# balint256/gr-baz

Measured on AMD Instinct MI355X. Metric: MUSIC-DoA snapshots/s (4 ant, 1024 samp, 3600 bins), higher is better.
Workload: dtype f64; 1 GPU; cfg2 (BASELINE.json configs[1]): m=4 n=2 nsamples=1024 (K=256) resolution=3600, spectrum port wired, 8 streams x 32768 items per GPU per step, device-resident; streams_total=8, items_per_launch_sequence=262144, parallelism=independent streams, s mod 1, no collective, collective_backend_fell_back=False

## Files before the change

### gr_baz_amd/csrc/baz_music_hip.hip

```cpp
#include "../../include/baz_music_hip.h"
#include "music_kernels.hip.h"
#include "music_wide_kernels.hip.h"
#include "scan_coarse_kernels.hip.h"
#include "scan_i8_kernels.hip.h"
#ifdef BAZ_MUSIC_LAB
#include "scan_i8p_kernels.hip.h"
#include "sort_kernels.hip.h"
#endif
#include "table_kernels.hip.h"
#include "smoothing_kernels.hip.h"
#include "refine_kernels.hip.h"
#include "average_kernels.hip.h"

#include <algorithm>
#include <chrono>
#include <cmath>
#include <cstdio>
#include <cstdlib>
#include <cstring>
#include <unistd.h>
#include <mutex>
#include <thread>
#include <new>
#include <string>
// ... 174 lines not shown
    uint32_t wide_cap = 0;
    double* dSs = nullptr;
    int sig_scan = 1;
    uint8_t* dRedo = nullptr;
    int sub_evd = 1;
    int fused_covevd = 0;
    uint32_t covevd_blocks = 512u;
    int covevd_task_items = 0;
    uint32_t cov4_resident_blocks = 256u;
    uint32_t cs_tiles = 0;
    int coarse = 1;
    int coarse_rg = 4;
    int coarse_lab = 0;
    int coarse_stats = 0;
    unsigned long long* dMargin = nullptr;
#ifdef BAZ_MUSIC_LAB
    uint16_t* dKeys = nullptr;
    uint32_t* dHist = nullptr;
    uint32_t* dCursor = nullptr;
    uint32_t* dPerm = nullptr;
    uint32_t sort_cap = 0;
    unsigned long long* dFire = nullptr;
    unsigned long long* hFire = nullptr;
    unsigned long long* hFireDev = nullptr;
    unsigned long long fire_calls = 0, fire_seen = 0;
    int sort_mode = 0;
    bool sort_on = false;
    uint32_t sort_streak = 0;
    uint64_t sort_clock = 0, sort_retry_at = 0;
    double rate_unsorted = 0.0;
    uint64_t sorted_calls = 0, unsorted_calls = 0;
#endif
    uint32_t scan_lds_pad = 0;
    int seq_walk = 0;
#ifdef BAZ_MUSIC_LAB
    int i8p_on = 0;
#endif
    int i8_on = 1;
    int i8_abl = 0;
    int refine_nocount = 0;
    uint32_t num_cus = 256;
    int i8_wgs_per_cu[2][2][2] = {{{0, 0}, {0, 0}}, {{0, 0}, {0, 0}}};
    unsigned long long* dI8Stat = nullptr;
    int peak_mode = 0;
    float* dPeakSpec = nullptr;
    size_t peak_spec_cap = 0;
    int order_mode = 0;
    uint32_t order_nsnap = 0;
    uint8_t* dOrd = nullptr;
    size_t ord_cap = 0;
    uint32_t ord_count = 0;
    uint32_t ord_items = 0;
    bool ord_on = false;
    bool ord_driven = false;
    uint8_t* ord_cur = nullptr;
    uint8_t* dOrdTap = nullptr;
    size_t ord_tap_cap = 0;
    int refine_mode = 0;
    float* dRefAl = nullptr;
    size_t ref_al_cap = 0;
    double* dRefOff = nullptr;
    size_t ref_off_cap = 0;
    uint32_t ref_count = 0;
    bool ref_on = false;
    uint32_t avg_window = 1;
    double avg_beta = 1.0;
    double avg_neff = 1.0;
    bazavg::AvgTable avg_tab = {};
    uint32_t avg_hist = 0;
    int avg_parity = 0;
    double2* dAvgHist[2] = {nullptr, nullptr};
    size_t avg_hist_cap[2] = {0, 0};
    double2* dRavg = nullptr;
    size_t ravg_cap = 0;
    size_t chunk_bytes = 0;
    struct HostPin { uintptr_t lo, hi; uint32_t asked; };
    std::vector<HostPin> pins;
    std::vector<HostPin> refused;
    uint64_t pinned_bytes = 0;
    uint64_t pin_limit = 4096ull << 20;
    int auto_pin = 0;
    int zero_copy = 1;
    int single_limit_mib = 64;
    StageProf prof[BAZ_MUSIC_NUM_STAGES];
    std::string stage_name[BAZ_MUSIC_NUM_STAGES];
    char scan_names[4][64] = {{0}, {0}, {0}, {0}};
    int scan_kind = -1;
    char hip_err[256] = {0};
    struct Smoothing {
        baz_music_ctx* inner = nullptr;
        uint32_t ms = 0, L = 1, Kp = 0;
        int fb = 0;
        bazsmooth::Perm perm = {};
        float2* dY = nullptr;
        size_t y_cap = 0;
        float* dX = nullptr;
        float* dAl = nullptr;
        float* dSpec = nullptr;
        size_t x_cap = 0, al_cap = 0, spec_cap = 0;
    } sm;
};

namespace {

int hip_fail(baz_music_ctx* c, hipError_t e, const char* what)
{
    if (c) snprintf(c->hip_err, sizeof(c->hip_err), "%s: %s", what, hipGetErrorString(e));
    (void)hipGetLastError();
    return BAZ_MUSIC_E_HIP;
}

#define HIP_TRY(ctx, call)                                         \
    do {                                                           \
        hipError_t e__ = (call);                                   \
        if (e__ != hipSuccess) return hip_fail((ctx), e__, #call); \
    } while (0)

struct DeviceGuard {
    int prev = -1;
// ... 526 lines not shown

int launch_frontend(baz_music_ctx* c, const void* d_in, uint32_t batch, double* dQ, uint32_t qstride)
{
    const float* in = static_cast<const float*>(d_in);
    if (c->avg_window > 1) {
        int ra = launch_cov(c, in, batch, c->dR);
        if (ra == BAZ_MUSIC_OK) ra = launch_average(c, c->dR, batch, c->dRavg);
        return ra ? ra : launch_evd(c, c->dRavg, batch, dQ, qstride, c->dG);
    }
    if (c->fused_covevd) return launch_covevd(c, in, batch, dQ, qstride, c->dG);
    const int r = launch_cov(c, in, batch, c->dR);
    return r ? r : launch_evd(c, c->dR, batch, dQ, qstride, c->dG);
}

uint32_t topn_list_len(uint32_t n) { return n <= 2 ? 2u : (n <= 4 ? 4u : (n <= 8 ? 8u : 16u)); }
uint32_t forced_nsplit(int force_nsplit, uint32_t most) { return std::max<uint32_t>(1u, std::min<uint32_t>((uint32_t)force_nsplit, most)); }

struct ScanGeom { uint32_t groups, nsplit, blocks, rows_per_class; };
constexpr uint32_t SCAN_WANT_TASKS = 256u * 4u * 4u * 2u;
constexpr uint32_t SCAN_MAX_NSPLIT = 64;
ScanGeom scan_geometry(uint32_t batch, uint32_t nsteps, uint32_t nclass, int force_nsplit, uint32_t m)
{
    ScanGeom G;
    G.rows_per_class = round_up((batch + nclass - 1) / nclass, 64);
    G.groups = nclass * (G.rows_per_class / 16);
    const uint32_t live_groups = (batch + 15) / 16;
    const uint32_t want_tasks = (m >= 9) ? SCAN_WANT_TASKS / 4u : SCAN_WANT_TASKS;
    const uint32_t ns = (want_tasks + live_groups - 1) / live_groups;
    G.nsplit = std::max<uint32_t>(1u, std::min<uint32_t>(ns, std::min<uint32_t>(nsteps, SCAN_MAX_NSPLIT)));
    if (force_nsplit > 0) G.nsplit = forced_nsplit(force_nsplit, std::min<uint32_t>(nsteps, SCAN_MAX_NSPLIT));
    G.blocks = (G.groups / 4) * G.nsplit;
    return G;
}
size_t scan_cand_ranges(const baz_music_ctx* c, uint32_t batch)
{
    const size_t cap_split = std::min<size_t>(SCAN_MAX_NSPLIT, std::max<uint32_t>(1u, c->fb_steps));
    const size_t exact = (size_t)batch * scan_geometry(batch, c->fb_steps, c->nclass, c->force_nsplit, c->m).nsplit;
    const size_t worst = std::min<size_t>((size_t)batch * cap_split, (size_t)16u * SCAN_WANT_TASKS + (size_t)batch);
    const size_t forced = c->force_nsplit > 0 ? (size_t)batch * forced_nsplit(c->force_nsplit, (uint32_t)cap_split) : 0;
    return std::max(std::max(exact, worst), std::max(forced, (size_t)batch));
}

constexpr uint32_t I8_MAX_NSPLIT = 16, I8_MAX_ROUNDS = 8;
uint32_t i8_nsplit(uint32_t batch, uint32_t nsteps, uint32_t slots, int force_nsplit)
{
    const uint32_t groups = std::max<uint32_t>(1u, (batch + 63) / 64);
    const uint32_t cap = std::max<uint32_t>(1u, std::min<uint32_t>(I8_MAX_NSPLIT, nsteps / 4));
    if (force_nsplit > 0) return forced_nsplit(force_nsplit, std::min<uint32_t>(nsteps, SCAN_MAX_NSPLIT));
    uint32_t best = 1;
    double best_fill = 0.0;
    for (uint32_t r = 1; r <= I8_MAX_ROUNDS; ++r) {
        const uint32_t ns = std::max<uint32_t>(1u, std::min<uint32_t>(cap, (uint32_t)(((uint64_t)r * slots) / groups)));
        const uint64_t blocks = (uint64_t)groups * ns;
        const uint64_t rounds = (blocks + slots - 1) / slots;
        const double fill = (double)blocks / (double)(rounds * slots);
        if (fill > best_fill * 1.03) { best_fill = fill; best = ns; }
        if (ns == cap) break;
    }
    return best;
}
size_t i8_cand_ranges(const baz_music_ctx* c, uint32_t batch)
{
    if (!c->tab.dIB) return 0;
    const size_t exact = (size_t)batch * (c->force_nsplit > 0 ? forced_nsplit(c->force_nsplit, SCAN_MAX_NSPLIT) : I8_MAX_NSPLIT);
    return std::max(exact, std::min<size_t>((size_t)batch * I8_MAX_NSPLIT, (size_t)64u * I8_MAX_ROUNDS * 4u * c->num_cus + (size_t)batch));
}
// ... 98 lines not shown
}

template <int M>
int launch_sort_t(baz_music_ctx* c, const double* dQ, uint32_t qstride, uint32_t batch)
{
    if constexpr (M <= 8) {
        const uint32_t ns = bazsort::key_samples(c->res);
        const uint32_t padded = round_up(batch, 256);
        hipLaunchKernelGGL((bazsort::coarse_key_kernel<M>), dim3(padded / 256), dim3(256), 0, c->stream, dQ, c->tab.dKT, ns, batch, qstride, c->dKeys);
        HIP_TRY(c, hipGetLastError());
        hipLaunchKernelGGL((bazsort::key_sweep_kernel<false>), dim3(bazsort::KEY_BLOCKS), dim3(256), 0, c->stream, c->dKeys, padded / 8, c->dHist,
                           c->dCursor, c->dPerm);
        HIP_TRY(c, hipGetLastError());
        hipLaunchKernelGGL((bazsort::key_sweep_kernel<true>), dim3(bazsort::KEY_BLOCKS), dim3(256), 0, c->stream, c->dKeys, padded / 8, c->dHist,
                           c->dCursor, c->dPerm);
        HIP_TRY(c, hipGetLastError());
    }
    return BAZ_MUSIC_OK;
}
#endif

ScanRefine scan_refine(const baz_music_ctx* c, bool a2)
{
    ScanRefine rf;
    rf.Gs = c->refine_off ? nullptr : c->dG;
    rf.TB = c->tab.dTB + c->tb_step_elems;
    rf.below = c->tab.refine_below;
    rf.count = c->refine_nocount ? nullptr : c->dRefined + c->stat_parity;
    rf.A2 = (a2 && c->tab.dA2p) ? c->tab.dA2p + 64 : nullptr;
    return rf;
}
ScanRefine scan_refine_validation(const baz_music_ctx* c) { return {nullptr, c->tab.dTB + c->tb_step_elems, 0.0, nullptr, nullptr}; }

enum ScanKind { SCAN_FP64 = 0, SCAN_I8 = 1, SCAN_COARSE = 2, SCAN_I8P = 3 };
struct ScanForm { ScanKind kind; bool short_form; };

ScanForm scan_form(const baz_music_ctx* c, bool spec)
{
    if (!spec && coarse_applies(c) && !c->order_mode) return {SCAN_COARSE, false};
    if (spec && i8p_active(c)) return {SCAN_I8P, false};
    const bool gated_shape = c->m <= 8 && !short_form_applies(c->m, c->n);
    if (i8_active(c) && (spec || !gated_shape)) return {SCAN_I8, false};
    return {SCAN_FP64, short_form_in_use(c)};
}

struct ScanCall { uint32_t batch, qstride; float* spec; bool vec4; };

struct ScanDone {
    int rc;
    ScanKind kind;
    uint32_t nsplit;
#ifdef BAZ_MUSIC_LAB
    bool sorted = false;
#endif
};
ScanDone scan_result(baz_music_ctx* c, ScanDone done, int rc) { done.rc = rc; if (rc == BAZ_MUSIC_OK) c->scan_kind = done.kind; return done; }
int launch_rc(baz_music_ctx* c) { HIP_TRY(c, hipGetLastError()); return BAZ_MUSIC_OK; }
ScanDone scan_no_kernel(ScanKind kind) { return {BAZ_MUSIC_E_UNSUPPORTED, kind, 1}; }
struct CoarseLaunch {
    uint32_t blocks, nphases, nsplit;
    ScanRefine rf;
    unsigned long long* stats;
    float* val_dump = nullptr;
    const uint32_t* perm = nullptr;
    unsigned long long* fstat = nullptr;
};
template <int M, typename Kernel>
void coarse_launch(baz_music_ctx* c, Kernel kernel, const CoarseLaunch& L, uint32_t batch, uint32_t qstride)
{
    hipLaunchKernelGGL(kernel, dim3(L.blocks), dim3(256), 0, c->stream, c->dQ, c->tab.dCS, c->tab.dCS + (size_t)(c->cs_tiles + 1) * cs_c_units(M),
                       c->dCand, batch, c->res, qstride, L.nphases, L.nsplit, c->keep_mask, c->n, L.rf, c->tab.cs, L.stats, L.val_dump, L.perm, L.fstat);
}

struct I8Launch {
    uint32_t blocks, nsplit, n;
    float* spec;
// ... 100 lines not shown
        ScanDone done{BAZ_MUSIC_OK, SCAN_I8P, G.nsplit};
        if ((size_t)s.batch * G.nsplit * NMAX > c->cand_cap) return scan_result(c, done, BAZ_MUSIC_E_INVALID);
        const I8Launch L{G.blocks, G.nsplit, c->n, s.spec, scan_refine(c, false), c->dI8Stat, nullptr};
        auto* kernel = s.vec4 ? &scan_i8p_kernel<M, NMAX, true, true> : &scan_i8p_kernel<M, NMAX, true, false>;
        if constexpr (M == 4 && NMAX == 2) {
            if (s.vec4 && c->i8_abl) {
                switch (c->i8_abl) {
                    case 1: kernel = &scan_i8p_kernel<M, NMAX, true, true, false, 1>; break;
                    case 2: kernel = &scan_i8p_kernel<M, NMAX, true, true, false, 2>; break;
                    case 4: kernel = &scan_i8p_kernel<M, NMAX, true, true, false, 4>; break;
                    case 5: kernel = &scan_i8p_kernel<M, NMAX, true, true, false, 5>; break;
                    default: kernel = &scan_i8p_kernel<M, NMAX, true, true, false, 3>; break;
                }
            }
        }
        i8p_launch(c, kernel, L, G.rows_per_class, s.batch, s.qstride);
        return scan_result(c, done, launch_rc(c));
    }
    return scan_no_kernel(SCAN_I8P);
}
#else
template <int M, int NMAX>
ScanDone launch_scan_i8p(baz_music_ctx*, const ScanCall&) { return scan_no_kernel(SCAN_I8P); }
#endif

template <int M, int NMAX, int SIG>
auto* scan_fp64_kernel(const ScanCall& s)
{
    if (s.vec4) return &scan_mfma_kernel<M, NMAX, true, true, 0, (1 | 2 | 16), SIG>;
    if (s.spec) return &scan_mfma_kernel<M, NMAX, true, false, 0, (1 | 2 | 16), SIG>;
    return &scan_mfma_kernel<M, NMAX, false, false, 0, (1 | 2 | 16), SIG>;
}

template <int M, int NMAX>
ScanDone launch_scan_fp64(baz_music_ctx* c, const ScanCall& s, bool short_form)
{
    const ScanGeom G = scan_geometry(s.batch, c->fb_steps, c->nclass, c->force_nsplit, c->m);
    ScanDone done{BAZ_MUSIC_OK, SCAN_FP64, G.nsplit};
    if ((size_t)s.batch * G.nsplit * NMAX > c->cand_cap) return scan_result(c, done, BAZ_MUSIC_E_INVALID);
    auto* kernel = scan_fp64_kernel<M, NMAX, 0>(s);
    if constexpr (M >= 6 && NMAX == 2) {
        if (short_form && c->n == 1) kernel = scan_fp64_kernel<M, NMAX, 1>(s);
        if constexpr (M >= 9) if (short_form && c->n == 2) kernel = scan_fp64_kernel<M, NMAX, 2>(s);
    }
#ifdef BAZ_MUSIC_LAB
    if constexpr (M == 4 && NMAX == 2) {
        if (s.vec4 && c->lab_variant) {
            switch (c->lab_variant) {
                case 2: kernel = &scan_mfma_kernel<M, NMAX, true, true, 64, (1 | 2 | 16)>; break;
                case 3: kernel = &scan_mfma_kernel<M, NMAX, true, true, 0, 0>; break;
                case 4: kernel = &scan_mfma_kernel<M, NMAX, true, true, 0, 2>; break;
                case 5: kernel = &scan_mfma_kernel<M, NMAX, true, true, 0, (1 | 16)>; break;
                case 6: kernel = &scan_mfma_kernel<M, NMAX, true, true, 1, (1 | 2 | 16)>; break;
                case 7: kernel = &scan_mfma_kernel<M, NMAX, true, true, (8 | 2 | 4), (1 | 2 | 16)>; break;
                case 8: kernel = &scan_mfma_kernel<M, NMAX, true, true, (1 | 2), (1 | 2 | 16)>; break;
                case 9: kernel = &scan_mfma_kernel<M, NMAX, true, true, 1024, (1 | 2 | 16)>; break;
                case 10: kernel = &scan_mfma_kernel<M, NMAX, true, true, (1024 | 2048), (1 | 2 | 16)>; break;
                case 11: kernel = &scan_mfma_kernel<M, NMAX, true, true, 2048, (1 | 2 | 16)>; break;
                case 12: kernel = &scan_mfma_kernel<M, NMAX, true, true, 4096, (1 | 2 | 16)>; break;
                case 13: kernel = &scan_mfma_kernel<M, NMAX, true, true, (8 | 2 | 4 | 4096), (1 | 2 | 16)>; break;
                case 14: kernel = &scan_mfma_kernel<M, NMAX, true, true, 8192, (1 | 2 | 16)>; break;
                case 15: kernel = &scan_mfma_kernel<M, NMAX, true, true, 16384, (1 | 2 | 16)>; break;
                default: break;
            }
        }
    }
#endif
    const double* coeff = short_form ? c->dSs : c->dQ;
    const double2* image = short_form ? c->tab.dTB + c->tb_step_elems : c->tab.dFB + c->fb_step_elems;
    hipLaunchKernelGGL(kernel, dim3(G.blocks), dim3(256), short_form ? 0 : (size_t)c->scan_lds_pad, c->stream, coeff, image, s.spec, c->dCand, s.batch,
                       c->res, s.qstride, G.nsplit, c->nclass, G.rows_per_class, c->keep_mask, scan_n(c), scan_refine(c, true), (uint32_t)c->seq_walk);
    return scan_result(c, done, launch_rc(c));
}

template <int M, int NMAX>
ScanDone launch_scan_t(baz_music_ctx* c, ScanForm form, const ScanCall& s)
{
    switch (form.kind) {
        case SCAN_COARSE: return launch_scan_coarse<M, NMAX>(c, s);
        case SCAN_I8P: return launch_scan_i8p<M, NMAX>(c, s);
        case SCAN_I8: return launch_scan_i8<M, NMAX>(c, s);
        default: return launch_scan_fp64<M, NMAX>(c, s, form.short_form);
    }
}

template <int M>
ScanDone launch_scan_m(baz_music_ctx* c, ScanForm form, const ScanCall& s)
{
    if (c->n <= 2) return launch_scan_t<M, 2>(c, form, s);
    if (c->n <= 4) return launch_scan_t<M, 4>(c, form, s);
    if constexpr (M > 5) {
        if (c->n <= 8) return launch_scan_t<M, 8>(c, form, s);
    }
    if constexpr (M > 9) return launch_scan_t<M, 16>(c, form, s);
    return scan_no_kernel(form.kind);
}

ScanDone launch_scan(baz_music_ctx* c, uint32_t qstride, uint32_t batch, float* d_spec)
{
    ProfScope ps(c, BAZ_MUSIC_STAGE_SCAN);
    const ScanForm form = scan_form(c, d_spec != nullptr);
    const ScanCall s{batch, qstride, d_spec, d_spec && (c->res % 4u) == 0 && (reinterpret_cast<uintptr_t>(d_spec) % 16u) == 0};
#define BAZ_CALL(MV) launch_scan_m<MV>(c, form, s)
    switch (c->m) {
        BAZ_M_CASES(BAZ_CALL)
        default: return scan_no_kernel(form.kind);
    }
#undef BAZ_CALL
}

int launch_merge(baz_music_ctx* c, const ScanDone& scan, uint32_t batch, float* d_ang, float* d_lvl, float* d_spec)
{
    ProfScope ps(c, BAZ_MUSIC_STAGE_MERGE);
    auto* kernel = &topn_merge_kernel<16>;
    switch (topn_list_len(c->n)) {
// ... 1079 lines not shown
            uint32_t gcd = 64;
            while (resolution % gcd) gcd >>= 1;
            c->nclass = 64u / gcd;
        }
        if (const char* v = BAZ_LAB_ENV("BAZ_MUSIC_NO_ROWCLASS")) { if (atoi(v)) c->nclass = 1; }
        if (const char* v = BAZ_LAB_ENV("BAZ_MUSIC_NO_REFINE")) c->refine_off = atoi(v);
        if (const char* v = BAZ_LAB_ENV("BAZ_MUSIC_NO_REFINE_COUNT")) c->refine_nocount = atoi(v);
        if (const char* v = BAZ_LAB_ENV("BAZ_MUSIC_COV_OLD")) c->lab_cov_old = atoi(v);
        if (const char* v = BAZ_LAB_ENV("BAZ_MUSIC_SUB_EVD")) c->sub_evd = atoi(v);
        if (const char* v = BAZ_LAB_ENV("BAZ_MUSIC_NSPLIT")) c->force_nsplit = std::max(0, atoi(v));
        {
            int fuse = 1;
            if (const char* v = BAZ_LAB_ENV("BAZ_MUSIC_FUSE")) fuse = atoi(v);
            if (const char* v = BAZ_LAB_ENV("BAZ_MUSIC_SCAN_LDS_PAD")) c->scan_lds_pad = (uint32_t)std::max(0, atoi(v));
            c->fused_covevd = (fuse > 0 && m == 4 && (c->K % 256u) == 0 && !c->lab_cov_old) ? 1 : 0;
            int per_cu = 0;
            if (hipOccupancyMaxActiveBlocksPerMultiprocessor(&per_cu, cov4_evd_kernel, 256, 0) == hipSuccess && per_cu > 0)
                c->covevd_blocks = (uint32_t)per_cu * (uint32_t)std::max(1, prop.multiProcessorCount);
            else (void)hipGetLastError();
        }
        if (const char* v = BAZ_LAB_ENV("BAZ_MUSIC_SIG_SCAN")) c->sig_scan = atoi(v);
        if (const char* v = getenv("BAZ_MUSIC_COARSE")) c->coarse = atoi(v);
        if (const char* v = BAZ_LAB_ENV("BAZ_MUSIC_COARSE_RG")) c->coarse_rg = atoi(v);
        if (const char* v = BAZ_LAB_ENV("BAZ_MUSIC_COARSE_LAB")) c->coarse_lab = atoi(v);
        if (const char* v = BAZ_LAB_ENV("BAZ_MUSIC_COARSE_STATS")) c->coarse_stats = atoi(v);
        if (m <= 8) {
            c->cs_tiles = round_up((resolution + 15) / 16, 8);
            if (dev_malloc((void**)&c->dMargin, sizeof(unsigned long long)) != hipSuccess) { r = BAZ_MUSIC_E_NOMEM; break; }
            if (hipMemsetAsync(c->dMargin, 0, sizeof(unsigned long long), c->stream) != hipSuccess) { r = BAZ_MUSIC_E_HIP; break; }
        }
        if (const char* v = getenv("BAZ_MUSIC_EXACT")) c->i8_on = atoi(v) ? 0 : 1;
        if (const char* v = BAZ_LAB_ENV("BAZ_MUSIC_I8_ABL")) c->i8_abl = atoi(v);
        if (const char* v = BAZ_LAB_ENV("BAZ_MUSIC_SEQ_WALK")) c->seq_walk = atoi(v) ? 1 : 0;
#ifdef BAZ_MUSIC_LAB
        if (const char* v = BAZ_LAB_ENV("BAZ_MUSIC_SORT")) c->sort_mode = atoi(v) < 0 ? -1 : (atoi(v) ? 1 : 0);
        if (const char* v = BAZ_LAB_ENV("BAZ_MUSIC_I8P")) c->i8p_on = atoi(v) ? 1 : 0;
#endif
        if (const char* v = BAZ_LAB_ENV("BAZ_MUSIC_COVEVD_TASK_ITEMS")) { const int t = atoi(v); c->covevd_task_items = (t == 64 || t == 32 || t == 16) ? t : 0; }
        bool wants_i8_stat = wants_i8_image(c);
#ifdef BAZ_MUSIC_LAB
        wants_i8_stat = wants_i8_stat || (c->i8p_on && m <= 4 && n <= 4);
#endif
        if (wants_i8_stat) {
            if (dev_malloc((void**)&c->dI8Stat, 8 * sizeof(unsigned long long)) != hipSuccess) { r = BAZ_MUSIC_E_NOMEM; break; }
            if (hipMemsetAsync(c->dI8Stat, 0, 8 * sizeof(unsigned long long), c->stream) != hipSuccess) { r = BAZ_MUSIC_E_HIP; break; }
        }
        {
            c->cov4_resident_blocks = (uint32_t)std::max(1, prop.multiProcessorCount);
            c->num_cus = (uint32_t)std::max(1, prop.multiProcessorCount);
            if (const char* v = BAZ_LAB_ENV("BAZ_MUSIC_COV_BLOCKS_PER_CU"))
                if (atoi(v) > 0) c->cov4_resident_blocks = (uint32_t)atoi(v) * (uint32_t)std::max(1, prop.multiProcessorCount);
        }
        if (dev_malloc((void**)&c->dRefined, 2 * sizeof(unsigned long long)) != hipSuccess) { r = BAZ_MUSIC_E_NOMEM; break; }
        if (hipMemsetAsync(c->dRefined, 0, 2 * sizeof(unsigned long long), c->stream) != hipSuccess) { r = BAZ_MUSIC_E_HIP; break; }
        r = create_tables(c, table_ri);
    } while (0);
    if (r != BAZ_MUSIC_OK) {
        baz_music_destroy(c);
        return r;
    }
    if (wide) {
        c->stage_name[BAZ_MUSIC_STAGE_COV] = !c->wide_cov_mfma ? "bazwide::cov_wide_kernel" : (m > 32 ? "bazwide::cov_wide_pairs_kernel" : "bazwide::cov_wide_mfma_kernel");
        c->stage_name[BAZ_MUSIC_STAGE_EVD] = "bazwide::evd_wide_kernel";
        c->stage_name[BAZ_MUSIC_STAGE_SCAN] = c->wide_mfma ? "bazwide::scan_wide_mfma_kernel" : "bazwide::scan_wide_kernel";
        c->stage_name[BAZ_MUSIC_STAGE_MERGE] = c->wide_mfma ? (n <= 2 ? "bazmusic::topn_merge_kernel<2>" : (n <= 4 ? "bazmusic::topn_merge_kernel<4>" : "bazmusic::topn_merge_kernel<8>")) : "bazwide::topn_wide_kernel";
        *out = c;
        return BAZ_MUSIC_OK;
    }
    char buf[128];
    snprintf(buf, sizeof(buf), m <= 8 ? "bazmusic::cov_mfma_kernel<%u>" : "bazmusic::cov_mfma2_kernel<%u>", m);
    c->stage_name[BAZ_MUSIC_STAGE_COV] = buf;
    if (m == 4 && (c->K % 256u) == 0 && !c->lab_cov_old) c->stage_name[BAZ_MUSIC_STAGE_COV] = "bazmusic::cov4_x4_kernel";
    if (c->fused_covevd) c->stage_name[BAZ_MUSIC_STAGE_COV] = "bazmusic::cov4_evd_kernel";
    snprintf(buf, sizeof(buf), m <= 4 ? "bazmusic::evd_proj_kernel<%u>" : "bazmusic::evd_proj_lds_kernel<%u>", m);
    c->stage_name[BAZ_MUSIC_STAGE_EVD] = buf;
    snprintf(buf, sizeof(buf), "bazmusic::topn_merge_kernel<%u>", topn_list_len(n));
    c->stage_name[BAZ_MUSIC_STAGE_MERGE] = buf;
    static const char* const scan_kernels[4] = {"scan_mfma_kernel", "scan_i8_kernel", "scan_coarse_kernel", "scan_i8p_kernel"};
    for (int k = 0; k < 4; ++k) snprintf(c->scan_names[k], sizeof(c->scan_names[k]), "bazmusic::%s<%u,", scan_kernels[k], m);
    *out = c;
    return BAZ_MUSIC_OK;
}

void baz_music_destroy(baz_music_ctx* c)
{
    if (!c) return;
    {
        DeviceGuard guard(c->device);
        if (c->sm.inner) baz_music_destroy(c->sm.inner);
        c->sm.inner = nullptr;
        if (c->stream) (void)hipStreamSynchronize(c->stream);
        free_smoothing_buffers(c);
        for (auto& p : c->prof)
            for (auto e : p.ev) (void)hipEventDestroy(e);
        if (c->h_al_big) (void)hipHostFree(c->h_al_big);
        if (c->s_tab) (void)hipStreamSynchronize(c->s_tab);
        free_table_set(c->tab);
        free_table_set(c->shadow);
        if (c->dRaw) (void)dev_free(c->dRaw);
        if (c->hRaw) (void)hipHostFree(c->hRaw);
        if (c->dTabStats) (void)dev_free(c->dTabStats);
        if (c->hTabStats) (void)hipHostFree(c->hTabStats);
        if (c->ev_swap) (void)hipEventDestroy(c->ev_swap);
        if (c->s_tab) (void)hipStreamDestroy(c->s_tab);
#ifdef BAZ_MUSIC_LAB
        if (c->dKeys) (void)dev_free(c->dKeys);
        if (c->dPerm) (void)dev_free(c->dPerm);
        if (c->dHist) (void)dev_free(c->dHist);
        if (c->dCursor) (void)dev_free(c->dCursor);
        if (c->dFire) (void)dev_free(c->dFire);
        if (c->hFire) (void)hipHostFree(c->hFire);
#endif
// ... 1104 lines not shown
```

### gr_baz_amd/csrc/music_kernels.hip.h

```cpp
#pragma once

#include <hip/hip_runtime.h>
#include <stdint.h>

#include "order_kernels.hip.h"

namespace bazmusic {

typedef double v4f64 __attribute__((ext_vector_type(4)));
typedef float v4f32 __attribute__((ext_vector_type(4)));
typedef uint32_t v4u32 __attribute__((ext_vector_type(4)));
typedef double v2f64 __attribute__((ext_vector_type(2)));

__device__ __forceinline__ void wave_lds_fence()
{
    __builtin_amdgcn_fence(__ATOMIC_RELEASE, "wavefront");
    __builtin_amdgcn_wave_barrier();
    __builtin_amdgcn_fence(__ATOMIC_ACQUIRE, "wavefront");
}

template <int M>
__global__ __launch_bounds__(256) void cov_mfma_kernel(const float* __restrict__ in,
                                                        double2* __restrict__ R,
                                                        uint32_t batch, uint32_t K)
// ... 878 lines not shown
            for (int part = 0; part < 2; ++part) {
                v4f64 p = {0, 0, 0, 0};
                const int comp = part ? ((g & 1) ^ 1) : (g & 1);
                const double sgn = (part && !(g & 1)) ? -1.0 : 1.0;
                const double* __restrict__ ga = rf.Gs + (size_t)((k * M + (g >> 1)) * 2 + comp) * qstride + itc;
                const double* __restrict__ tb = tb1 + (size_t)(t >> 1) * 128 + (t & 1);
                if constexpr (KS2 <= 2) {
#pragma unroll
                    for (int s = 0; s < KS2; ++s) {
                        const double a = (4 * s + g < 2 * M) ? sgn * ga[(size_t)s * 4 * qstride] : 0.0;
                        p = __builtin_amdgcn_mfma_f64_16x16x4f64(a, tb[(size_t)s * 256], p, 0, 0, 0);
                    }
                } else {
#pragma nounroll
                    for (int s = 0; s < KS2; ++s) {
                        const double a = (4 * s + g < 2 * M) ? sgn * ga[(size_t)s * 4 * qstride] : 0.0;
                        p = __builtin_amdgcn_mfma_f64_16x16x4f64(a, tb[(size_t)s * 256], p, 0, 0, 0);
                    }
                }
                d += p * p;
            }
        }
#pragma unroll
        for (int r = 0; r < 4; ++r) {
            const bool redo = (fabs(acc[t][r]) <= rf.below) && (bin + t < res);
            acc[t][r] = redo ? d[r] : acc[t][r];
            cnt += (redo && row_ok[r]) ? 1u : 0u;
        }
        __builtin_amdgcn_sched_barrier(0);
    }
    return cnt;
}

template <int M, int NMAX, bool SPEC, bool VEC4, int ABL = 0, int AUX = (1 | 2 | 16), int SIG = 0>
__global__ __launch_bounds__(256, (M <= 4 && NMAX <= 2) ? ((ABL & 2048) ? 3 : 4) : (M >= 9 ? 2 : 1)) void scan_mfma_kernel(const double* __restrict__ Qs,
                                                         const double2* __restrict__ FB,
                                                         float* __restrict__ spec,
                                                         double* __restrict__ cand,
                                                         uint32_t batch, uint32_t res, uint32_t qstride,
                                                         uint32_t nsplit, uint32_t nclass, uint32_t rows_per_class,
                                                         uint32_t keep_mask, uint32_t n, ScanRefine rf, uint32_t seq_walk = 0)
{
    constexpr int MM = M * M;
    constexpr int KS = SIG ? (2 * M + 3) / 4 : (MM + 3) / 4;
    static_assert(!SIG || (((SIG == 1 && M >= 6) || M >= 9) && KS <= 8), "the short form: one phase per step, no row classes (m >= 6)");
    constexpr int NG = (SIG == 1) ? 2 : 4;
    constexpr int SCH = (KS <= 8) ? KS : 8;
    constexpr int PPS = (KS + SCH - 1) / SCH;
    constexpr int CPP = 2 * SCH;
    constexpr int SPW = (CPP + 3) / 4;
    __shared__ v2f64 stage[2][CPP * 64];

    const int lane = threadIdx.x & 63;
    const int wave = __builtin_amdgcn_readfirstlane(threadIdx.x >> 6);
    const int c = lane & 15, g = lane >> 4;

    const uint32_t split = blockIdx.x % nsplit;
    const uint32_t blk = blockIdx.x / nsplit;
    uint32_t p0;
    if constexpr ((ABL & 4096) == 0) p0 = (blk * 4 + wave) * 16;
    else p0 = (blk % nclass) * rows_per_class + ((blk / nclass) * 4 + wave) * 16;
    const uint32_t cls = __builtin_amdgcn_readfirstlane(p0 / rows_per_class);
    const uint32_t j0 = p0 - cls * rows_per_class;
    const uint32_t sh = ((res & 63u) * cls) & 63u;
    const int shc = (int)(sh >> 2);
    const uint32_t nsteps = (res + sh + 63u) >> 6;
    const uint32_t st_begin = (uint32_t)(((uint64_t)nsteps * split) / nsplit);
    const uint32_t st_end = (uint32_t)(((uint64_t)nsteps * (split + 1)) / nsplit);
    const uint32_t item0 = nclass * j0 + cls;

    double qa[SIG ? 1 : KS];
    [[maybe_unused]] double sa[SIG ? NG : 1][SIG ? KS : 1];
    const uint32_t it_c = item0 + nclass * (uint32_t)c;
    const uint32_t itc = (it_c < batch) ? it_c : (batch - 1);
    if constexpr (SIG) {
#pragma unroll
        for (int q = 0; q < NG; ++q) {
            const int sub = c >> 2;
            const int wrow = (SIG == 1) ? (c & 3) + 4 * (2 * q + (sub >> 1)) : (c & 3) + 4 * q;
            const int outp = (SIG == 1) ? (sub & 1) : sub;
            const uint32_t it_q = item0 + nclass * (uint32_t)wrow;
            const uint32_t itq = (it_q < batch) ? it_q : (batch - 1);
#pragma unroll
            for (int s = 0; s < KS; ++s) {
                const int e = 4 * s + g;
                sa[q][s] = (e < 2 * M) ? Qs[(size_t)(outp * 2 * M + e) * qstride + itq] : 0.0;
            }
        }
        qa[0] = 0.0;
    } else {
#pragma unroll
        for (int s = 0; s < KS; ++s) {
            const int e = 4 * s + g;
// ... 29 lines not shown
#define BAZ_FB_LD(IDX) ((ABL & 256) ? __builtin_nontemporal_load(fb + (IDX)) : fb[(IDX)])
#define BAZ_STAGE_DMA(ST, P, BUF)                                                                \
    do {                                                                                         \
        if (wave4 == (int)(turn & 3u)) {                                                         \
            const int nch__ = 2 * ((KS - (P) * SCH < SCH) ? (KS - (P) * SCH) : SCH);             \
            const size_t ch0__ = ((size_t)(ST) * KS + (size_t)(P) * SCH) * 2;                    \
            _Pragma("unroll")                                                                    \
            for (int j__ = 0; j__ < CPP; ++j__)                                                  \
                if (j__ < nch__)                                                                 \
                    __builtin_amdgcn_global_load_lds((const __attribute__((address_space(1))) void*)(fb + (ch0__ + j__) * 64), \
                                                     (__attribute__((address_space(3))) void*)(&stage[(BUF)][j__ * 64]), 16, 0, 0); \
        }                                                                                        \
    } while (0)
#define BAZ_STAGE_LOAD(ST, P)                                                                    \
    do {                                  \
        if constexpr (!(ABL & 128)) {                                                            \
        const int nch__ = 2 * ((KS - (P) * SCH < SCH) ? (KS - (P) * SCH) : SCH);                 \
        const size_t ch0__ = ((size_t)(ST) * KS + (size_t)(P) * SCH) * 2;                        \
        sreg0 = BAZ_FB_LD((ch0__ + (wave4 < nch__ ? wave4 : nch__ - 1)) * 64);                   \
        if constexpr (SPW > 1) sreg1 = BAZ_FB_LD((ch0__ + (wave4 + 4 < nch__ ? wave4 + 4 : nch__ - 1)) * 64);   \
        if constexpr (SPW > 2) sreg2 = BAZ_FB_LD((ch0__ + (wave4 + 8 < nch__ ? wave4 + 8 : nch__ - 1)) * 64);   \
        if constexpr (SPW > 3) sreg3 = BAZ_FB_LD((ch0__ + (wave4 + 12 < nch__ ? wave4 + 12 : nch__ - 1)) * 64); \
        }                                                                                        \
    } while (0)
#define BAZ_STAGE_STORE(BUF, P)                                                                  \
    do {                                                                                         \
        const int nch__ = 2 * ((KS - (P) * SCH < SCH) ? (KS - (P) * SCH) : SCH);                 \
        if (wave4 < nch__) stage[(BUF)][wave4 * 64 + lane] = sreg0;                              \
        if constexpr (SPW > 1) { if (wave4 + 4 < nch__) stage[(BUF)][(wave4 + 4) * 64 + lane] = sreg1; }   \
        if constexpr (SPW > 2) { if (wave4 + 8 < nch__) stage[(BUF)][(wave4 + 8) * 64 + lane] = sreg2; }   \
        if constexpr (SPW > 3) { if (wave4 + 12 < nch__) stage[(BUF)][(wave4 + 12) * 64 + lane] = sreg3; } \
    } while (0)

    if (st_begin < st_end) {
        if constexpr (ROT) {
            BAZ_STAGE_DMA(st_begin, 0, 0);
            asm volatile("s_waitcnt vmcnt(0)" ::: "memory");
            ++turn;
        } else {
            BAZ_STAGE_LOAD(st_begin, 0);
            BAZ_STAGE_STORE(0, 0);
        }
    }
    __syncthreads();

    int buf = 0;
    v4f32 sv[4] = {{0, 0, 0, 0}, {0, 0, 0, 0}, {0, 0, 0, 0}, {0, 0, 0, 0}};
    float* __restrict__ spec_base = SPEC ? spec + (size_t)item0 * res - sh : nullptr;
    uint32_t soff0 = 0;
    const uint32_t row4 = 4u * nclass * res * 4u;
    [[maybe_unused]] __amdgpu_buffer_rsrc_t spec_rsrc = __builtin_amdgcn_make_buffer_rsrc(spec_base, 0, 0x7FFFFFFF, 0x00020000);
    bool row_ok[4];
#pragma unroll
    for (int r = 0; r < 4; ++r) {
        if (r == 0) soff0 = ((uint32_t)g * nclass * res + 4u * (uint32_t)c) * 4u;
        row_ok[r] = (item0 + nclass * (uint32_t)(g + 4 * r)) < batch;
    }
    const uint32_t nst = st_end - st_begin;
    const uint32_t SW = seq_walk ? 1u : (nst >= 64u ? 8u : (nst >= 16u ? 4u : (nst >= 6u ? 2u : 1u)));
    uint32_t st = st_begin, sweep = 0;
    for (uint32_t it = 0; it < nst; ++it) {
        uint32_t st_next = st + SW, sweep_next = sweep;
        if (st_next >= st_end) { sweep_next = sweep + 1; st_next = st_begin + sweep_next; }
        const bool has_next = it + 1 < nst;
        v4f64 acc[4];
#pragma unroll
        for (int t = 0; t < 4; ++t) acc[t] = (v4f64){0, 0, 0, 0};
        const uint32_t bin = st * 64 + 4 * c - sh;

#pragma unroll
        for (int p = 0; p < PPS; ++p) {
            const bool last_p = (p == PPS - 1);
            const bool more = !last_p || has_next;
            if constexpr (ROT) { if (more) BAZ_STAGE_DMA(last_p ? st_next : st, last_p ? 0 : p + 1, buf ^ 1); }
            else { if (more) BAZ_STAGE_LOAD(last_p ? st_next : st, last_p ? 0 : p + 1); }

            if constexpr (SIG) {
                const v4f64 a2v = *reinterpret_cast<const v4f64*>(rf.A2 + (size_t)st * 64 + 4 * c);
#pragma unroll
                for (int q = 0; q < NG; ++q) {
                    v4f64 tmp[4];
#pragma unroll
                    for (int t = 0; t < 4; ++t) tmp[t] = (v4f64){0, 0, 0, 0};
#pragma unroll
                    for (int sl = 0; sl < KS; ++sl) {
                        const v2f64 f01 = stage[buf][(2 * sl) * 64 + lane];
                        const v2f64 f23 = stage[buf][(2 * sl + 1) * 64 + lane];
                        tmp[0] = __builtin_amdgcn_mfma_f64_16x16x4f64(sa[q][sl], f01.x, tmp[0], 0, 0, 0);
                        tmp[1] = __builtin_amdgcn_mfma_f64_16x16x4f64(sa[q][sl], f01.y, tmp[1], 0, 0, 0);
                        tmp[2] = __builtin_amdgcn_mfma_f64_16x16x4f64(sa[q][sl], f23.x, tmp[2], 0, 0, 0);
                        tmp[3] = __builtin_amdgcn_mfma_f64_16x16x4f64(sa[q][sl], f23.y, tmp[3], 0, 0, 0);
                    }
#pragma unroll
                    for (int t = 0; t < 4; ++t) {
                        if constexpr (SIG == 1) {
                            acc[t][2 * q] = a2v[t] - (tmp[t][0] * tmp[t][0] + tmp[t][1] * tmp[t][1]);
                            acc[t][2 * q + 1] = a2v[t] - (tmp[t][2] * tmp[t][2] + tmp[t][3] * tmp[t][3]);
                        } else {
                            acc[t][q] = a2v[t] - ((tmp[t][0] * tmp[t][0] + tmp[t][1] * tmp[t][1]) +
                                                  (tmp[t][2] * tmp[t][2] + tmp[t][3] * tmp[t][3]));
                        }
                    }
                }
            } else {
            if constexpr (ABL & 8192) __builtin_amdgcn_s_setprio(3);
            if constexpr (ABL & 16384) __builtin_amdgcn_s_setprio(0);
#pragma unroll
            for (int sl = 0; sl < SCH; ++sl) {
                const int s = p * SCH + sl;
                if (s < KS) {
                    const v2f64 f01 = stage[buf][(2 * sl) * 64 + lane];
                    const v2f64 f23 = stage[buf][(2 * sl + 1) * 64 + lane];
                    if constexpr (ABL & 8) {
                        acc[0][s & 3] += qa[s] * f01.x; acc[1][s & 3] += qa[s] * f01.y;
                        acc[2][s & 3] += qa[s] * f23.x; acc[3][s & 3] += qa[s] * f23.y;
                    } else {
                        acc[0] = __builtin_amdgcn_mfma_f64_16x16x4f64(qa[s], f01.x, acc[0], 0, 0, 0);
                        acc[1] = __builtin_amdgcn_mfma_f64_16x16x4f64(qa[s], f01.y, acc[1], 0, 0, 0);
                        acc[2] = __builtin_amdgcn_mfma_f64_16x16x4f64(qa[s], f23.x, acc[2], 0, 0, 0);
                        acc[3] = __builtin_amdgcn_mfma_f64_16x16x4f64(qa[s], f23.y, acc[3], 0, 0, 0);
                    }
                }
            }
            if constexpr (ABL & 8192) __builtin_amdgcn_s_setprio(0);
            if constexpr (ABL & 16384) __builtin_amdgcn_s_setprio(3);
            }

            if (last_p) {
#pragma unroll
                for (int r = 0; r < 4; ++r) asm volatile("" ::"v"(sv[r]));
                bool hit = false, low = false;
#pragma unroll
                for (int r = 0; r < 4; ++r) {
                    if constexpr (SPEC && !(ABL & 4)) {
                        float fd[4];
#pragma unroll
                        for (int t = 0; t < 4; ++t) fd[t] = (float)acc[t][r];
                        if constexpr (!(ABL & 2)) {
                            float mn;
                            asm("v_min3_f32 %0, |%1|, |%2|, |%3|" : "=v"(mn) : "v"(fd[0]), "v"(fd[1]), "v"(fd[2]));
                            asm("v_min_f32 %0, %1, |%2|" : "=v"(mn) : "v"(mn), "v"(fd[3]));
                            hit |= (mn <= gate_f[r]);
                            low |= (mn <= below_f);
                        }
#pragma unroll
// ... 55 lines not shown
            } else {
                if (more) BAZ_STAGE_STORE(buf ^ 1, last_p ? 0 : p + 1);
            }

            if (last_p) {
                if constexpr (ABL & 1) {
#pragma unroll
                    for (int r = 0; r < 4; ++r) asm volatile("" ::"v"(sv[r]));
                }
                if constexpr (SPEC && !(ABL & 1)) {
                    const int step_off = (int)(st * 256u);
                    if constexpr (VEC4) {
                        if ((st > 0 || sh == 0) && st * 64 + 64 - sh <= res) {
#pragma unroll
                            for (int r = 0; r < 4; ++r)
                                if (row_ok[r]) __builtin_amdgcn_raw_buffer_store_b128(__builtin_bit_cast(v4u32, sv[r]), spec_rsrc, (int)soff0, step_off + (int)(row4 * (uint32_t)r), AUX);
                        } else {
#pragma unroll
                            for (int r = 0; r < 4; ++r)
                                if (row_ok[r] && bin < res) __builtin_amdgcn_raw_buffer_store_b128(__builtin_bit_cast(v4u32, sv[r]), spec_rsrc, (int)soff0, step_off + (int)(row4 * (uint32_t)r), AUX);
                        }
                    } else {
#pragma unroll
                        for (int r = 0; r < 4; ++r) {
                            const v4u32 u = __builtin_bit_cast(v4u32, sv[r]);
#pragma unroll
                            for (int t = 0; t < 4; ++t)
                                if (row_ok[r] && bin + t < res)
                                    __builtin_amdgcn_raw_buffer_store_b32(u[t], spec_rsrc, (int)(soff0 + 4u * t), step_off + (int)(row4 * (uint32_t)r), AUX);
                        }
                    }
                }
            }
            if constexpr (ROT) {
                asm volatile("s_waitcnt lgkmcnt(0)" ::: "memory");
                __builtin_amdgcn_s_barrier();
                asm volatile("" ::: "memory");
            } else {
                __syncthreads();
            }
            buf ^= 1;
        }
        st = st_next;
        sweep = sweep_next;
    }

    if (rf.count && lane == 0 && refined_wave) atomicAdd(rf.count, (unsigned long long)refined_wave);
#pragma unroll
    for (int r = 0; r < 4; ++r) {
        key_merge_xor<NMAX>(key[r], 1);
        key_merge_xor<NMAX>(key[r], 2);
        key_merge_xor<NMAX>(key[r], 4);
        key_merge_xor<NMAX>(key[r], 8);
        const uint32_t it = item0 + nclass * (uint32_t)(g + 4 * r);
        if (c == 0 && it < batch) {
#pragma unroll
            for (int i = 0; i < NMAX; ++i) cand[((size_t)it * nsplit + split) * NMAX + i] = key[r][i];
        }
    }
}

#undef BAZ_STAGE_LOAD
#undef BAZ_STAGE_DMA
#undef BAZ_FB_LD
#undef BAZ_STAGE_STORE

template <int NMAX>
__global__ __launch_bounds__(256) void topn_merge_kernel(const double* __restrict__ cand,
                                                          const float* __restrict__ spec,
                                                          float* __restrict__ ang, float* __restrict__ lvl,
                                                          uint32_t batch, uint32_t res, uint32_t n, uint32_t nsplit,
                                                          uint32_t keep_mask, unsigned long long* __restrict__ next_stat,
                                                          unsigned long long* __restrict__ fire_dev = nullptr,
                                                          unsigned long long* __restrict__ fire_host = nullptr,
// ... 73 lines not shown
```

Before: 229.4 million snapshots/s.

## Add deep LDS ring-buffer scan form with 16-wave workgroups for small m

Adds a ring variant of the fp64 MFMA scan kernel for m<=4, n<=2 with the spectrum port wired. It uses one 16-wave workgroup per CU and a multi-chunk dynamic-LDS ring filled by global_load_lds DMA, waited on with counted vmcnt. This replaces the per-step double-buffer stage and its per-step barriers, aiming to hide steering-table fetch latency and cut sync overhead. It is chosen only when the staged geometry would not split and there are enough blocks to fill the CUs. The cost is large LDS use, lower occupancy flexibility, and fragile hand-counted wait logic.

```diff
diff --git a/gr_baz_amd/csrc/baz_music_hip.hip b/gr_baz_amd/csrc/baz_music_hip.hip
--- a/gr_baz_amd/csrc/baz_music_hip.hip
+++ b/gr_baz_amd/csrc/baz_music_hip.hip
@@ -230,6 +230,9 @@
     uint64_t sorted_calls = 0, unsorted_calls = 0;
 #endif
     uint32_t scan_lds_pad = 0;
+    int scan_ring = -1;
+    bool scan_ring_attr[2] = {false, false};
+    int scan_ring_lab = 0;
     int seq_walk = 0;
 #ifdef BAZ_MUSIC_LAB
     int i8p_on = 0;
@@ -282,7 +285,7 @@
     int single_limit_mib = 64;
     StageProf prof[BAZ_MUSIC_NUM_STAGES];
     std::string stage_name[BAZ_MUSIC_NUM_STAGES];
-    char scan_names[4][64] = {{0}, {0}, {0}, {0}};
+    char scan_names[5][64] = {{0}, {0}, {0}, {0}, {0}};
     int scan_kind = -1;
     char hip_err[256] = {0};
     struct Smoothing {
@@ -875,6 +878,20 @@
     G.blocks = (G.groups / 4) * G.nsplit;
     return G;
 }
+ScanGeom scan_geometry_ring(uint32_t batch, uint32_t nclass)
+{
+    ScanGeom G;
+    G.rows_per_class = round_up((batch + nclass - 1) / nclass, 256);
+    G.groups = nclass * (G.rows_per_class / 16);
+    G.nsplit = 1;
+    G.blocks = G.groups / 16;
+    return G;
+}
+bool scan_ring_taken(const baz_music_ctx* c, const ScanGeom& staged, const ScanGeom& ring)
+{
+    if (c->scan_ring == 1) return true;
+    return staged.nsplit == 1 && ring.blocks >= c->num_cus;
+}
 size_t scan_cand_ranges(const baz_music_ctx* c, uint32_t batch)
 {
     const size_t cap_split = std::min<size_t>(SCAN_MAX_NSPLIT, std::max<uint32_t>(1u, c->fb_steps));
@@ -1039,8 +1056,8 @@
 }
 ScanRefine scan_refine_validation(const baz_music_ctx* c) { return {nullptr, c->tab.dTB + c->tb_step_elems, 0.0, nullptr, nullptr}; }
 
-enum ScanKind { SCAN_FP64 = 0, SCAN_I8 = 1, SCAN_COARSE = 2, SCAN_I8P = 3 };
-struct ScanForm { ScanKind kind; bool short_form; };
+enum ScanKind { SCAN_FP64 = 0, SCAN_I8 = 1, SCAN_COARSE = 2, SCAN_I8P = 3, SCAN_FP64_RING = 4 };
+struct ScanForm { ScanKind kind; bool short_form; bool ring = false; };
 
 ScanForm scan_form(const baz_music_ctx* c, bool spec)
 {
@@ -1048,7 +1065,8 @@
     if (spec && i8p_active(c)) return {SCAN_I8P, false};
     const bool gated_shape = c->m <= 8 && !short_form_applies(c->m, c->n);
     if (i8_active(c) && (spec || !gated_shape)) return {SCAN_I8, false};
-    return {SCAN_FP64, short_form_in_use(c)};
+    const bool short_form = short_form_in_use(c);
+    return {SCAN_FP64, short_form, !short_form && spec && c->m <= 4 && c->n <= 2 && c->scan_ring != 0};
 }
 
 struct ScanCall { uint32_t batch, qstride; float* spec; bool vec4; };
@@ -1215,10 +1233,53 @@
     return &scan_mfma_kernel<M, NMAX, false, false, 0, (1 | 2 | 16), SIG>;
 }
 
+constexpr int SCAN_RING_C = 4, SCAN_RING_R = 12;
+template <int M, int RC, int RR, int RW = 16>
+int launch_scan_ring_t(baz_music_ctx* c, const ScanCall& s, const ScanGeom& G)
+{
+    constexpr int lds = RR * 2 * ((M * M + 3) / 4) * 1024;
+    auto* kernel = s.vec4 ? &scan_mfma_kernel<M, 2, true, true, 0, (1 | 2 | 16), 0, RC, RR, RW> : &scan_mfma_kernel<M, 2, true, false, 0, (1 | 2 | 16), 0, RC, RR, RW>;
+    if (!c->scan_ring_attr[s.vec4 ? 1 : 0]) {
+        HIP_TRY(c, hipFuncSetAttribute(reinterpret_cast<const void*>(kernel), hipFuncAttributeMaxDynamicSharedMemorySize, lds));
+        c->scan_ring_attr[s.vec4 ? 1 : 0] = true;
+    }
+    hipLaunchKernelGGL(kernel, dim3(G.blocks * (16 / RW)), dim3(RW * 64), (size_t)lds, c->stream, c->dQ, c->tab.dFB + c->fb_step_elems, s.spec, c->dCand, s.batch,
+                       c->res, s.qstride, G.nsplit, c->nclass, G.rows_per_class, c->keep_mask, scan_n(c), scan_refine(c, true), (uint32_t)c->seq_walk);
+    return launch_rc(c);
+}
+template <int M>
+int launch_scan_ring(baz_music_ctx* c, const ScanCall& s, const ScanGeom& G)
+{
+#ifdef BAZ_MUSIC_LAB
+    if constexpr (M == 4) {
+        switch (c->scan_ring_lab) {
+            case 1: return launch_scan_ring_t<M, 4, 8>(c, s, G);
+            case 2: return launch_scan_ring_t<M, 2, 8>(c, s, G);
+            case 3: return launch_scan_ring_t<M, 4, 16>(c, s, G);
+            case 4: return launch_scan_ring_t<M, 2, 6>(c, s, G);
+            case 5: return launch_scan_ring_t<M, 2, 6, 8>(c, s, G);
+            case 6: return launch_scan_ring_t<M, 4, 8, 8>(c, s, G);
+            default: break;
+        }
+    }
+#endif
+    return launch_scan_ring_t<M, SCAN_RING_C, SCAN_RING_R>(c, s, G);
+}
+
 template <int M, int NMAX>
-ScanDone launch_scan_fp64(baz_music_ctx* c, const ScanCall& s, bool short_form)
+ScanDone launch_scan_fp64(baz_music_ctx* c, const ScanCall& s, bool short_form, bool ring)
 {
     const ScanGeom G = scan_geometry(s.batch, c->fb_steps, c->nclass, c->force_nsplit, c->m);
+    if constexpr (M <= 4 && NMAX == 2) {
+        if (ring && s.spec && !short_form) {
+            const ScanGeom GR = scan_geometry_ring(s.batch, c->nclass);
+            if (scan_ring_taken(c, G, GR)) {
+                ScanDone done{BAZ_MUSIC_OK, SCAN_FP64_RING, GR.nsplit};
+                if ((size_t)s.batch * NMAX > c->cand_cap) return scan_result(c, done, BAZ_MUSIC_E_INVALID);
+                return scan_result(c, done, launch_scan_ring<M>(c, s, GR));
+            }
+        }
+    }
     ScanDone done{BAZ_MUSIC_OK, SCAN_FP64, G.nsplit};
     if ((size_t)s.batch * G.nsplit * NMAX > c->cand_cap) return scan_result(c, done, BAZ_MUSIC_E_INVALID);
     auto* kernel = scan_fp64_kernel<M, NMAX, 0>(s);
@@ -1263,7 +1324,7 @@
         case SCAN_COARSE: return launch_scan_coarse<M, NMAX>(c, s);
         case SCAN_I8P: return launch_scan_i8p<M, NMAX>(c, s);
         case SCAN_I8: return launch_scan_i8<M, NMAX>(c, s);
-        default: return launch_scan_fp64<M, NMAX>(c, s, form.short_form);
+        default: return launch_scan_fp64<M, NMAX>(c, s, form.short_form, form.ring);
     }
 }
 
@@ -2409,6 +2470,8 @@
         if (const char* v = getenv("BAZ_MUSIC_EXACT")) c->i8_on = atoi(v) ? 0 : 1;
         if (const char* v = BAZ_LAB_ENV("BAZ_MUSIC_I8_ABL")) c->i8_abl = atoi(v);
         if (const char* v = BAZ_LAB_ENV("BAZ_MUSIC_SEQ_WALK")) c->seq_walk = atoi(v) ? 1 : 0;
+        if (const char* v = BAZ_LAB_ENV("BAZ_MUSIC_SCAN_RING")) c->scan_ring = atoi(v) ? 1 : 0;
+        if (const char* v = BAZ_LAB_ENV("BAZ_MUSIC_SCAN_RING_GEOM")) c->scan_ring_lab = atoi(v);
 #ifdef BAZ_MUSIC_LAB
         if (const char* v = BAZ_LAB_ENV("BAZ_MUSIC_SORT")) c->sort_mode = atoi(v) < 0 ? -1 : (atoi(v) ? 1 : 0);
         if (const char* v = BAZ_LAB_ENV("BAZ_MUSIC_I8P")) c->i8p_on = atoi(v) ? 1 : 0;
@@ -2455,6 +2518,7 @@
     c->stage_name[BAZ_MUSIC_STAGE_MERGE] = buf;
     static const char* const scan_kernels[4] = {"scan_mfma_kernel", "scan_i8_kernel", "scan_coarse_kernel", "scan_i8p_kernel"};
     for (int k = 0; k < 4; ++k) snprintf(c->scan_names[k], sizeof(c->scan_names[k]), "bazmusic::%s<%u,", scan_kernels[k], m);
+    snprintf(c->scan_names[SCAN_FP64_RING], sizeof(c->scan_names[SCAN_FP64_RING]), "bazmusic::scan_mfma_kernel<%u,ring>", m);
     *out = c;
     return BAZ_MUSIC_OK;
 }
diff --git a/gr_baz_amd/csrc/music_kernels.hip.h b/gr_baz_amd/csrc/music_kernels.hip.h
--- a/gr_baz_amd/csrc/music_kernels.hip.h
+++ b/gr_baz_amd/csrc/music_kernels.hip.h
@@ -934,8 +934,17 @@
     return cnt;
 }
 
-template <int M, int NMAX, bool SPEC, bool VEC4, int ABL = 0, int AUX = (1 | 2 | 16), int SIG = 0>
-__global__ __launch_bounds__(256, (M <= 4 && NMAX <= 2) ? ((ABL & 2048) ? 3 : 4) : (M >= 9 ? 2 : 1)) void scan_mfma_kernel(const double* __restrict__ Qs,
+template <int DMA, int ST, int P, int I = 0>
+__device__ __forceinline__ void ring_wait(const int idx)
+{
+    if constexpr (I < P * (P + 1)) {
+        if (idx == I) asm volatile("s_waitcnt vmcnt(%0)" ::"n"(DMA * (I / (P + 1)) + ST * (I % (P + 1))) : "memory");
+        else ring_wait<DMA, ST, P, I + 1>(idx);
+    }
+}
+
+template <int M, int NMAX, bool SPEC, bool VEC4, int ABL = 0, int AUX = (1 | 2 | 16), int SIG = 0, int RC = 0, int RR = 0, int RW = 16>
+__global__ __launch_bounds__(RC ? RW * 64 : 256, RC ? 16 / RW : ((M <= 4 && NMAX <= 2) ? ((ABL & 2048) ? 3 : 4) : (M >= 9 ? 2 : 1))) void scan_mfma_kernel(const double* __restrict__ Qs,
                                                          const double2* __restrict__ FB,
                                                          float* __restrict__ spec,
                                                          double* __restrict__ cand,
@@ -951,7 +960,16 @@
     constexpr int PPS = (KS + SCH - 1) / SCH;
     constexpr int CPP = 2 * SCH;
     constexpr int SPW = (CPP + 3) / 4;
-    __shared__ v2f64 stage[2][CPP * 64];
+    constexpr bool RING = RC > 0;
+    static_assert(!RING || (!SIG && SPEC && ABL == 0 && PPS == 1 && M <= 4 && NMAX <= 2), "the ring form: projector form, m <= 4, n <= 2, spectrum port");
+    static_assert(!RING || (RR % RC == 0 && RR / RC >= 2 && RR / RC <= 4), "the ring: 2 .. 4 whole chunks");
+    static_assert(RW == 16 || RW == 8, "the ring form: one 16-wave workgroup per CU (lab: two of 8 waves)");
+    constexpr int WPB = RING ? RW : 4;
+    constexpr int RCS = RING ? RR / RC : 2;
+    constexpr int RPC = RING ? CPP * RC : 16;
+    constexpr int RDW = (RPC + WPB - 1) / WPB;
+    __shared__ v2f64 stage[RING ? 1 : 2][RING ? 1 : CPP * 64];
+    extern __shared__ v2f64 ring[];
 
     const int lane = threadIdx.x & 63;
     const int wave = __builtin_amdgcn_readfirstlane(threadIdx.x >> 6);
@@ -960,7 +978,7 @@
     const uint32_t split = blockIdx.x % nsplit;
     const uint32_t blk = blockIdx.x / nsplit;
     uint32_t p0;
-    if constexpr ((ABL & 4096) == 0) p0 = (blk * 4 + wave) * 16;
+    if constexpr ((ABL & 4096) == 0) p0 = (blk * WPB + wave) * 16;
     else p0 = (blk % nclass) * rows_per_class + ((blk / nclass) * 4 + wave) * 16;
     const uint32_t cls = __builtin_amdgcn_readfirstlane(p0 / rows_per_class);
     const uint32_t j0 = p0 - cls * rows_per_class;
@@ -1056,6 +1074,7 @@
         if constexpr (SPW > 3) { if (wave4 + 12 < nch__) stage[(BUF)][(wave4 + 12) * 64 + lane] = sreg3; } \
     } while (0)
 
+    if constexpr (!RING) {
     if (st_begin < st_end) {
         if constexpr (ROT) {
             BAZ_STAGE_DMA(st_begin, 0, 0);
@@ -1067,6 +1086,7 @@
         }
     }
     __syncthreads();
+    }
 
     int buf = 0;
     v4f32 sv[4] = {{0, 0, 0, 0}, {0, 0, 0, 0}, {0, 0, 0, 0}, {0, 0, 0, 0}};
@@ -1083,7 +1103,66 @@
     const uint32_t nst = st_end - st_begin;
     const uint32_t SW = seq_walk ? 1u : (nst >= 64u ? 8u : (nst >= 16u ? 4u : (nst >= 6u ? 2u : 1u)));
     uint32_t st = st_begin, sweep = 0;
+
+    [[maybe_unused]] uint32_t fst = st_begin, fsweep = 0, fpos = 0;
+    [[maybe_unused]] uint32_t fslot = 0;
+    [[maybe_unused]] uint32_t rfetched = 0;
+    [[maybe_unused]] uint32_t rchunk = 0, rcpos = 0, rslot = 0;
+    [[maybe_unused]] const char* ring_src = reinterpret_cast<const char*>(FB) - (size_t)CPP * 1024;
+    [[maybe_unused]] const uint32_t ring_lds = RING ? (uint32_t)(uintptr_t)(__attribute__((address_space(3))) void*)(ring) : 0u;
+    [[maybe_unused]] const bool ring_counted = VEC4 && (item0 + nclass * 15u) < batch;
+    [[maybe_unused]] auto ring_fetch = [&]() {
+        uint32_t stq[RING ? RC : 1];
+#pragma unroll
+        for (int q = 0; q < RC; ++q) {
+            stq[q] = fst;
+            if (fpos + (uint32_t)q + 1u < nst) {
+                uint32_t nx = fst + SW;
+                if (nx >= st_end) { ++fsweep; nx = st_begin + fsweep; }
+                fst = nx;
+            }
+        }
+        fpos += RC;
+        uint32_t lq = (uint32_t)lane;
+        asm volatile("" : "+v"(lq));
+        const int cq = (int)(lq & 15u) - shc;
+        const uint32_t ring_voff = (((lq >> 4) * 16u + (uint32_t)(cq < 0 ? cq + 16 : cq)) + (cq < 0 ? 0u : (uint32_t)(CPP * 64))) * 16u;
+#pragma unroll
+        for (int i = 0; i < RDW; ++i) {
+            int j = wave + WPB * i;
+            j = j < RPC ? j : RPC - 1;
+            const int q = j / CPP, pc = j % CPP;
+            uint32_t s = stq[0];
+#pragma unroll
+            for (int qq = 1; qq < RC; ++qq) s = (q == qq) ? stq[qq] : s;
+            const char* src = ring_src + ((size_t)s * CPP + (size_t)pc) * 1024u;
+            const uint32_t dst = ring_lds + ((fslot * RC + (uint32_t)q) * CPP + (uint32_t)pc) * 1024u;
+            uint32_t keep;
+            asm volatile("s_nop 4\n\ts_mov_b32 %0, m0\n\ts_mov_b32 m0, %3\n\ts_nop 0\n\tglobal_load_lds_dwordx4 %1, %2\n\ts_mov_b32 m0, %0"
+                         : "=&s"(keep) : "v"(ring_voff), "s"(src), "s"(dst) : "memory");
+        }
+        fslot = (fslot + 1u == (uint32_t)RCS) ? 0u : fslot + 1u;
+        ++rfetched;
+    };
+    if constexpr (RING) {
+#pragma unroll
+        for (int k = 0; k < RCS - 1; ++k)
+            if (fpos < nst) ring_fetch();
+    }
+
     for (uint32_t it = 0; it < nst; ++it) {
+        if constexpr (RING) {
+            if (rcpos == 0) {
+                const int e = (int)(rfetched - 1u - rchunk), s = (int)(rchunk < (uint32_t)(RCS - 1) ? rchunk : (uint32_t)(RCS - 1));
+                if (ring_counted) ring_wait<RDW, 4 * RC, RCS - 1>(e * RCS + s);
+                else asm volatile("s_waitcnt vmcnt(0)" ::: "memory");
+                asm volatile("s_waitcnt lgkmcnt(0)" ::: "memory");
+                __builtin_amdgcn_s_barrier();
+                asm volatile("" ::: "memory");
+                if (fpos < nst) ring_fetch();
+            }
+        }
+        const v2f64* __restrict__ stg = RING ? ring + (size_t)rslot * (CPP * 64) : nullptr;
         uint32_t st_next = st + SW, sweep_next = sweep;
         if (st_next >= st_end) { sweep_next = sweep + 1; st_next = st_begin + sweep_next; }
         const bool has_next = it + 1 < nst;
@@ -1095,9 +1174,13 @@
 #pragma unroll
         for (int p = 0; p < PPS; ++p) {
             const bool last_p = (p == PPS - 1);
-            const bool more = !last_p || has_next;
+            const bool more = !RING && (!last_p || has_next);
             if constexpr (ROT) { if (more) BAZ_STAGE_DMA(last_p ? st_next : st, last_p ? 0 : p + 1, buf ^ 1); }
             else { if (more) BAZ_STAGE_LOAD(last_p ? st_next : st, last_p ? 0 : p + 1); }
+            auto stage_at = [&](const int idx) -> v2f64 {
+                if constexpr (RING) return stg[idx];
+                else return stage[buf][idx];
+            };
 
             if constexpr (SIG) {
                 const v4f64 a2v = *reinterpret_cast<const v4f64*>(rf.A2 + (size_t)st * 64 + 4 * c);
@@ -1133,8 +1216,8 @@
             for (int sl = 0; sl < SCH; ++sl) {
                 const int s = p * SCH + sl;
                 if (s < KS) {
-                    const v2f64 f01 = stage[buf][(2 * sl) * 64 + lane];
-                    const v2f64 f23 = stage[buf][(2 * sl + 1) * 64 + lane];
+                    const v2f64 f01 = stage_at((2 * sl) * 64 + lane);
+                    const v2f64 f23 = stage_at((2 * sl + 1) * 64 + lane);
                     if constexpr (ABL & 8) {
                         acc[0][s & 3] += qa[s] * f01.x; acc[1][s & 3] += qa[s] * f01.y;
                         acc[2][s & 3] += qa[s] * f23.x; acc[3][s & 3] += qa[s] * f23.y;
@@ -1256,7 +1339,8 @@
                     }
                 }
             }
-            if constexpr (ROT) {
+            if constexpr (RING) {
+            } else if constexpr (ROT) {
                 asm volatile("s_waitcnt lgkmcnt(0)" ::: "memory");
                 __builtin_amdgcn_s_barrier();
                 asm volatile("" ::: "memory");
@@ -1264,6 +1348,10 @@
                 __syncthreads();
             }
             buf ^= 1;
+        }
+        if constexpr (RING) {
+            rslot = (rslot + 1u == (uint32_t)RR) ? 0u : rslot + 1u;
+            if (++rcpos == (uint32_t)RC) { rcpos = 0; ++rchunk; }
         }
         st = st_next;
         sweep = sweep_next;
```

After: 228.1 million snapshots/s. Within noise of the previous version (-0.5%).
